# araray/sygnals

Hardware: AMD Instinct MI355X
Metric: Msamples/s STFT->MFCC (n_fft=2048, hop=512) (higher is better)
Workload: dtype f32; 1 GPU; C2: 1024 x 1 s @ 48 kHz clips per GPU, STFT n_fft=2048 hop=512 hann center -> 40-band Slaney mel -> power_to_db(ref=max, top_db=80) -> 13 MFCC (DCT-II ortho); clips_per_gpu=1024, clip_samples=48000, sr=48000, n_fft=2048, hop=512, n_mels=40, n_mfcc=13, rows_per_clip=13, parallelism=clip-sharded x1

## Files before the change

### sygnals_amd/core/features/manager.py

```python
from __future__ import annotations

import logging
from typing import Any, Dict, List, Optional

import numpy as np
import torch

from ... import _tables as T
from ... import ops
from ..._lib import SygnalsHipError

logger = logging.getLogger(__name__)

_SPECTRUM_BASED = ("spectral_centroid", "spectral_bandwidth", "spectral_flatness", "spectral_rolloff",
                   "dominant_frequency")
_SPECTROGRAM_BASED = ("spectral_contrast",)
_MELSPEC_BASED = ("mfcc",)
_FRAME_BASED = ("mean_amplitude", "std_dev_amplitude", "skewness", "kurtosis", "peak_amplitude", "crest_factor",
                "signal_entropy", "zero_crossing_rate", "rms_energy")
_REFERENCE_ONLY = ("hnr", "jitter", "shimmer")
_DEVICE_FEATURES = set(_SPECTRUM_BASED) | set(_SPECTROGRAM_BASED) | set(_MELSPEC_BASED) | set(_FRAME_BASED)
_ALL_KNOWN_FEATURES = _DEVICE_FEATURES | set(_REFERENCE_ONLY)


# ... 193 lines not shown
    if features != ["all"]:
        unknown = [f for f in features if f not in _ALL_KNOWN_FEATURES]
        if unknown:
            raise ValueError(f"Unknown feature(s) requested: {unknown}. Available: {sorted(_ALL_KNOWN_FEATURES)}")
    if y.ndim != 1:
        raise ValueError("Input audio signal 'y' must be a 1D array.")
    if output_format not in ("dataframe", "dict_of_arrays"):
        raise ValueError(f"Unsupported output format: {output_format}. Choose 'dataframe' or 'dict_of_arrays'.")
    import pandas as pd
    empty = pd.DataFrame() if output_format == "dataframe" else {"time": np.array([], dtype=np.float64)}
    if ops.num_frames(len(y), frame_length, hop_length, center) <= 0:
        logger.warning("Signal is too short for the given frame/hop length and centering setting. No frames generated.")
        return empty
    res = extract_features_batch(y[None, :].astype(np.float32), sr, features, frame_length, hop_length, center, window,
                                 feature_params)
    final = {"time": res.pop("time")}
    for k, v in res.items():
        final[k] = np.asarray(v[0], dtype=np.float64)
    if len(final) <= 1:
        logger.warning("No features were successfully extracted or passed final checks.")
        return empty if output_format == "dataframe" else {"time": final["time"]}
    if output_format == "dict_of_arrays":
        return final
    idx = pd.to_timedelta(final.pop("time"), unit="s")
    df = pd.DataFrame(final, index=idx)
    df.index.name = "time"
    return df


def features_one_launch(y, sr, hop_length, center, window, n_mels, fmin, fmax, n_mfcc, smask, roll_percent, bw_p, cplan):
    if not (1 <= n_mfcc <= n_mels <= 127 and (smask or cplan is not None)):
        return None
    launch = ops.stft2048_features_tri(y, sr, hop_length, center, window, n_mels, fmin, fmax, n_mfcc, smask, roll_percent,
                                       bw_p, cplan)
    return launch() if launch else None


TRI_FEATURES_DEFAULT = True


def feature_block(y, sr: int, hop_length: int = 512, n_mels: int = 40, n_mfcc: int = 13, roll_percent: float = 0.85,
                  n_bands: int = 6, fmin_contrast: float = 200.0, quantile: float = 0.02, out=None, one_launch=None,
                  projection: str = "auto", tri_waves: int = 16):
    ops.require_gpu()
    B, L = y.shape
    Tn = ops.num_frames(L, 2048, hop_length, True)
    freqs = np.fft.rfftfreq(2048, 1.0 / sr)
    cplan = ops._cached(("cplan", float(sr), n_bands, float(fmin_contrast), float(quantile)),
                        lambda: T.contrast_plan(freqs, sr, n_bands, fmin_contrast, quantile))
    R = int(cplan[0])
    if out is None:
        out = torch.empty((B, n_mfcc + 2 + R, Tn), dtype=torch.float32, device=y.device)
    if one_launch not in (None, True, False, "segments"):
        raise ValueError("one_launch must be None, True, False or 'segments'")
    launch = None
    if one_launch or (one_launch is None and TRI_FEATURES_DEFAULT):
        stats = torch.empty((B, 8, Tn), dtype=torch.float32, device=y.device)
        launch = ops.stft2048_features_tri(y, sr, hop_length, True, "hann", n_mels, 0.0, None, n_mfcc, 1 | 8, roll_percent, 2.0,
                                           cplan, out, stats)
        if launch is None and one_launch:
            raise SygnalsHipError("feature_block: no one-launch form for this shape (two-pass piece table + the clip's mel matrix in LDS)")
    if launch:
        _, stats, cpv = launch()
        mel = dct = None
    else:
        mel, stats, cpv = ops.stft2048_mel(y, sr, hop_length, True, "hann", 2048, n_mels, 0.0, None, 1 | 8 | 32, roll_percent,
                                           2.0, cplan, projection, tri_waves)
        dct = ops.dct_dev(n_mfcc, n_mels)
    ops._call("syg_feature_block_f32", ops._ptr(mel), B, n_mels, Tn, ops._ptr(dct), n_mfcc, 1e-10, 80.0, ops._ptr(stats),
              float(sr) / 2048.0, ops._ptr(cpv), R, 1e-10, 80.0, ops._ptr(out))
    return out


def feature_block_dominant(y, sr, hop_length, n_mels, n_mfcc):
    cplan = T.contrast_plan(np.fft.rfftfreq(2048, 1.0 / sr), sr)
    R = int(cplan[0])
    launch = None
    if TRI_FEATURES_DEFAULT:
        shape = (y.shape[0], n_mfcc + 2 + R, ops.num_frames(y.shape[1], 2048, hop_length, True))
        launch = ops.stft2048_features_tri(y, sr, hop_length, True, "hann", n_mels, 0.0, None, n_mfcc, 1 | 8, 0.85, 2.0, cplan,
                                           torch.empty(shape, dtype=torch.float32, device=y.device),
                                           torch.empty((shape[0], 8, shape[2]), dtype=torch.float32, device=y.device))
    if launch:
        return ("stft2048_kernel<16,2,7> (16 waves, staged tiles, per-wave mel projection by segment sums, clip-resident MFCC "
                "+ centroid + rolloff + contrast tail means)", launch, n_mfcc + 2 + 2 * R)
    return ("stft2048_kernel<16,2,1> (16 waves, staged tiles, mel + centroid + rolloff + contrast tail means)",
            lambda: ops.stft2048_mel(y, sr, hop_length, True, "hann", 2048, n_mels, 0.0, None, 1 | 8, 0.85, 2.0, cplan),
            n_mels + 3 + 2 * R)
```

### sygnals_amd/csrc/stft_mel.hip

```cpp
#include "stft_host.h"
#include <stdlib.h>

#define SETPRIO(n) __builtin_amdgcn_s_setprio(n)
#include "stft_dev.h"

typedef float syg_v2f __attribute__((ext_vector_type(2)));
__device__ syg_v2f syg_raw_buffer_load_v2f(__amdgpu_buffer_rsrc_t rs, int voffset, int soffset, int aux) __asm("llvm.amdgcn.raw.ptr.buffer.load.v2f32");

namespace syg {
namespace {

constexpr int NFFT = 2048;
constexpr int MC = 1024;
constexpr int NBIN = 1025;
constexpr int MAXW = 16;
constexpr int P_STRIDE = 1090;
constexpr int SC_COMPLEX = 528;
constexpr int TW2_STRIDE = 18;
constexpr int TW2_FLOATS = 4 * TW2_STRIDE * 2;
constexpr int TW1_FLOATS = 15 * 64 * 2;

struct MelPlan {
  int steps;
  int n_groups;
// ... 257 lines not shown

template <int WAVES>
__device__ __forceinline__ void stage_tile(const float* yb, int clip_bytes, float* stage, int s_begin, int span,
                                           bool wide, int w, int lane) {
  typedef __attribute__((address_space(3))) void* lds_ptr;
  const auto rs = __builtin_amdgcn_make_buffer_rsrc(const_cast<float*>(yb), 0, clip_bytes, 0x00020000);
  if (wide) {
    const int n = (span + 255) >> 8;
    for (int c = w; c < n; c += WAVES)
      __builtin_amdgcn_raw_ptr_buffer_load_lds(rs, (lds_ptr)(stage + c * 256), 16, (s_begin + c * 256 + lane * 4) * 4,
                                               0, 0, 0);
  } else {
    const int n = (span + 63) >> 6;
    for (int c = w; c < n; c += WAVES)
      __builtin_amdgcn_raw_ptr_buffer_load_lds(rs, (lds_ptr)(stage + c * 64), 4, (s_begin + c * 64 + lane) * 4, 0, 0,
                                               0);
  }
}
__device__ __forceinline__ MfccArgs uni(const MfccArgs& a) {
  MfccArgs u;
  u.dct = uni(a.dct); u.lifter = uni(a.lifter); u.out = uni(a.out); u.n_mfcc = uni(a.n_mfcc);
  u.ref_is_max = uni(a.ref_is_max); u.ref_value = uni(a.ref_value); u.amin = uni(a.amin); u.top_db = uni(a.top_db);
  u.tp = uni(a.tp); u.rows_per_clip = uni(a.rows_per_clip);
  return u;
}

typedef __attribute__((address_space(3))) float* lds_fptr;
#include "mel_segments.h"

template <int WAVES>
__device__ __noinline__ void clip_dct(int clipmel_addr, int red_addr, int dct_addr, MfccArgs mfv, int n_mels_v, int T_v, int b_v,
                                      int w_v, int lane, int stride_v = WAVES) {
  const MfccArgs mf = uni(mfv);
  const int n_mels = uni(n_mels_v), T = uni(T_v), w = uni(w_v), stride = uni(stride_v);
  const int64_t b = uni(b_v);
  lds_fptr clipmel = (lds_fptr)(uintptr_t)(uint32_t)uni(clipmel_addr);
  lds_fptr red = (lds_fptr)(uintptr_t)(uint32_t)uni(red_addr);
  lds_fptr dctl = (lds_fptr)(uintptr_t)(uint32_t)uni(dct_addr);
  lds_fptr lifl = dctl + mf.n_mfcc * n_mels;
  float m = red[lane & (WAVES - 1)];
  m = fmaxf(m, dpp_f<DPP_QP_1032>(m));
  m = fmaxf(m, dpp_f<DPP_QP_2301>(m));
  m = fmaxf(m, dpp_f<DPP_ROW_HALF_MIRROR>(m));
  m = fmaxf(m, dpp_f<DPP_ROW_MIRROR>(m));
  constexpr float DB_PER_LOG2 = 3.01029995663981195f;
  const float ref = mf.ref_is_max ? m : fabsf(mf.ref_value);
  const float reflog = __builtin_amdgcn_logf(fmaxf(mf.amin, ref));
  const float flo = (mf.top_db >= 0.f) ? DB_PER_LOG2 * (__builtin_amdgcn_logf(fmaxf(mf.amin, m)) - reflog) - mf.top_db
                                       : -3.4e38f;
  const int ktiles = (mf.n_mfcc + 15) >> 4, ttiles = mf.tp >> 4;
  const int f = lane & 15, g = lane >> 4;
  for (int ot = w; ot < ktiles * ttiles; ot += stride) {
    const int kt = ot / ttiles, tq = ot - kt * ttiles;
    const int krow = kt * 16 + f, tcol = tq * 16 + f;
    v4f acc = {0.f, 0.f, 0.f, 0.f};
    for (int m0 = 0; m0 < n_mels; m0 += 16) {
      float a[4], bv[4];
#pragma unroll
      for (int i = 0; i < 4; ++i) {
        const int mm = m0 + 4 * i + g;
        const bool ok = mm < n_mels;
        a[i] = (krow < mf.n_mfcc && ok) ? dctl[krow * n_mels + mm] : 0.f;
        bv[i] = ok ? clipmel[mm * mf.tp + tcol] : 1.f;
      }
#pragma unroll
      for (int i = 0; i < 4; ++i) {
        const float db = fmaxf(DB_PER_LOG2 * (__builtin_amdgcn_logf(fmaxf(mf.amin, bv[i])) - reflog), flo);
        acc = __builtin_amdgcn_mfma_f32_16x16x4f32(a[i], db, acc, 0, 0, 0);
      }
    }
#pragma unroll
    for (int r = 0; r < 4; ++r) {
      const int k = kt * 16 + 4 * g + r;
      if (k < mf.n_mfcc && tcol < T) {
        float val = acc[r];
        if (mf.lifter) val *= lifl[k];
        mf.out[(b * mf.rows_per_clip + k) * (int64_t)T + tcol] = val;
      }
    }
  }
}

constexpr int HANDOVER_ROUNDS = 1 << 16;
typedef __attribute__((address_space(3))) int* lds_ctr;
__device__ __forceinline__ int handover_load(lds_ctr c) {
  return __builtin_amdgcn_readfirstlane(__hip_atomic_load(c, __ATOMIC_ACQUIRE, __HIP_MEMORY_SCOPE_WORKGROUP));
}
template <int PRIO_BACK>
__device__ __forceinline__ bool handover_wait(lds_ctr c, int target) {
  if (handover_load(c) >= target) return true;
  if (PRIO_BACK >= 0) SETPRIO(0);
  bool ok = false;
#pragma unroll 1
  for (int r = 0; r < HANDOVER_ROUNDS && !ok; ++r) {
    __builtin_amdgcn_s_sleep(8);
    ok = handover_load(c) >= target;
  }
  if (PRIO_BACK >= 0) SETPRIO(PRIO_BACK);
  return ok;
}
__device__ __forceinline__ void handover_add(lds_ctr c, int lane) {
  if (lane == 0) __hip_atomic_fetch_add(c, 1, __ATOMIC_RELEASE, __HIP_MEMORY_SCOPE_WORKGROUP);
}

template <int WAVES, bool SLAB = true, int NPASS = 2>
struct Lds {
  static constexpr int TILE_T = WAVES;
  static constexpr int O_P = (NPASS == 4) ? 16 : 0;
  static constexpr int P_FLOATS = O_P + TILE_T * P_STRIDE + 16;
  static constexpr int SLAB_FLOATS = SLAB ? WAVES * 16 * TILE_T : 0;
  static constexpr int SEG_WORDS = NPASS * (SEGTAB_WORDS / 2);
  static constexpr int CPL_FLOATS = SLAB ? 3 * SYG_MAX_BANDS + MTAB_INTS : SEG_WORDS + 3 * SYG_MAX_BANDS;
  static constexpr int STAGE_FLOATS = (WAVES - 1) * 512 + NFFT;
  static constexpr int O_SLAB = P_FLOATS;
  static constexpr int O_TW2 = O_SLAB + SLAB_FLOATS;
  static constexpr int O_TW1 = O_TW2 + TW2_FLOATS;
  static constexpr int O_CPL = O_TW1 + TW1_FLOATS;
  static constexpr int O_WIN = O_CPL + CPL_FLOATS;
  static constexpr int O_STAGE = O_WIN + NFFT;
  static constexpr int TOTAL = O_STAGE + STAGE_FLOATS;
  static_assert(SC_COMPLEX * 2 <= P_STRIDE, "exchange scratch must fit inside a power row");
  static_assert(O_TW2 % 4 == 0 && O_WIN % 4 == 0 && O_STAGE % 4 == 0 && O_CPL % 4 == 0, "16-byte aligned LDS sections");
};

enum class Mode : int {
  Mel = 0, MelRows = 1, Complex = 2, ClipMatrix = 3, ClipSeg = 6, ClipSegRows = 7,
  TileSeg4 = 8, TileSeg4Rows = 9, TileSeg2 = 10, TileSeg2Rows = 11,
};
enum class Proj { None, Matrix, Segments };
constexpr bool X2_MEL = true;

struct ModeTraits {
  Proj proj;
  int npass;
  bool clip;
  bool rowfn;
  bool complex_out;
  bool power4;
  bool relc;
  bool freerun;
  constexpr bool seg() const { return proj == Proj::Segments; }
  constexpr bool seg_tile() const { return seg() && !clip; }
  constexpr bool x2() const { return X2_MEL && power4; }
  constexpr int clip_matrices() const { return seg() ? 2 : 1; }
};
constexpr ModeTraits mode_traits(Mode m) {
  switch (m) {
    case Mode::Mel:          return {Proj::Matrix,   2, false, false, false, true,  false, false};
    case Mode::MelRows:      return {Proj::Matrix,   2, false, true,  false, false, false, false};
    case Mode::Complex:      return {Proj::None,     2, false, false, true,  false, false, false};
    case Mode::ClipMatrix:   return {Proj::Matrix,   2, true,  false, false, true,  false, false};
    case Mode::ClipSeg:      return {Proj::Segments, 2, true,  false, false, true,  false,  true};
    case Mode::ClipSegRows:  return {Proj::Segments, 2, true,  true,  false, false, true, false};
    case Mode::TileSeg4:     return {Proj::Segments, 4, false, false, false, true,  false, false};
    case Mode::TileSeg4Rows: return {Proj::Segments, 4, false, true,  false, false, false, false};
    case Mode::TileSeg2:     return {Proj::Segments, 2, false, false, false, true,  false, false};
    case Mode::TileSeg2Rows: return {Proj::Segments, 2, false, true,  false, false, false, false};
  }
  return {};
}
template <int WAVES, Mode MODE>
using ModeLds = Lds<WAVES, !mode_traits(MODE).seg(), mode_traits(MODE).npass>;

template <int WAVES, int LOAD, Mode MODE>
__global__ __launch_bounds__(WAVES * 64, 4) void stft2048_kernel(
    const float* __restrict__ y, int64_t L, int64_t ldy, int hop, int pad, int64_t T, int tiles_per_clip,
    int64_t total_tiles, int tiles_per_wg, const float2* __restrict__ win2, const float2* __restrict__ twid,
    const float* __restrict__ wpacked, MelPlan plan, int n_mels, float* __restrict__ mel_out, float binhz,
    float roll_percent, float bw_p, int smask, float* __restrict__ stats_out, ContrastPlan cplan,
    float* __restrict__ contrast_out, float2* __restrict__ cout, int dma_wide, MfccArgs mf) {
  constexpr ModeTraits M = mode_traits(MODE);
  constexpr bool TRI = M.seg(), TRIMEL = M.seg_tile();
  constexpr int NPASS = M.npass;
  constexpr int TRI_ROW_BASE = (NPASS == 4) ? TRI4_ROW_BASE : 0;
  typedef ModeLds<WAVES, MODE> LM;
  constexpr int SEG_WORDS = LM::SEG_WORDS;
  constexpr int NTHREADS = WAVES * 64;
  constexpr int TILE_T = WAVES;
  constexpr bool COMPLEX_OUT = M.complex_out, ROWFN = M.rowfn, CLIPM = M.clip, X2 = M.x2();
  constexpr bool FREERUN = (LOAD >= 3), NOMEET = (LOAD == 4);
  static_assert(!FREERUN || (M.freerun && WAVES == 16 && TRI && CLIPM && !ROWFN), "LOAD 3 / 4: the free-running forms of the mode");
  constexpr int FLOAD = FREERUN ? 3 : LOAD;
#ifdef SYG_DEV_NO_RELC
  constexpr bool RELC = false;
#else
  constexpr bool RELC = M.relc;
#endif
  constexpr float MELSC = X2 ? 0.25f : 1.f;
  extern __shared__ __attribute__((aligned(16))) float lds[];
  float* Pbuf = lds + LM::O_P;
  float* slab = lds + LM::O_SLAB;
  float2* tw2l = reinterpret_cast<float2*>(lds + LM::O_TW2);
  float2* tw1l = reinterpret_cast<float2*>(lds + LM::O_TW1);
  int* cpl = reinterpret_cast<int*>(lds + LM::O_CPL);
  int* cplc = TRI ? cpl + SEG_WORDS : cpl;
  float2* winl = reinterpret_cast<float2*>(lds + LM::O_WIN);
  float* stage = lds + LM::O_STAGE;
  float* clipmel = lds + (LOAD == 2 ? LM::TOTAL : LM::O_STAGE);
  float* tri_red = clipmel + 2 * n_mels * mf.tp;
  float* tri_dct = tri_red + 2 * WAVES;

  const int tid = threadIdx.x, lane = tid & 63;
  const int w = __builtin_amdgcn_readfirstlane(tid >> 6);

  const int64_t tile_begin = (int64_t)blockIdx.x * tiles_per_wg;
  const int64_t tile_end = (tile_begin + tiles_per_wg < total_tiles) ? tile_begin + tiles_per_wg : total_tiles;
  if (tile_begin >= tile_end) return;

  auto clip_of = [&](int64_t tile) { return (uint32_t)tile / (uint32_t)tiles_per_clip; };
  auto t0_of = [&](int64_t tile, uint32_t cq) {
    return (int64_t)((uint32_t)tile - cq * (uint32_t)tiles_per_clip) * TILE_T;
  };
  const int span = (TILE_T - 1) * hop + NFFT;
  auto dma = [&](int64_t tile) {
    const uint32_t cq = clip_of(tile);
    int ld = lane;
    asm volatile("" : "+v"(ld));
    stage_tile<WAVES>(y + (int64_t)cq * ldy, (int)(L * 4), stage, (int)(t0_of(tile, cq) * hop) - pad, span,
                      dma_wide != 0, w, ld);
  };
  if (LOAD == 2) dma(tile_begin);

  LaneConst lc;
  init_lane_const(lc, lane, twid);
  float* prow = Pbuf + w * P_STRIDE;
  float2* sc = reinterpret_cast<float2*>(prow);
  if (tid < 64) tw2l[(tid >> 4) * TW2_STRIDE + (tid & 15)] = twid[32 * (tid >> 4) * (tid & 15)];
  for (int i = tid; i < 15 * 64; i += NTHREADS) tw1l[i] = twid[2 * (i & 63) * ((i >> 6) + 1)];
  for (int i = tid; i < NFFT / 2; i += NTHREADS) winl[i] = win2[i];
  if (CLIPM) {
    if (TRI)
      for (int i = tid; i < 2 * n_mels * mf.tp; i += NTHREADS) clipmel[i] = 0.f;
    float* dctl = TRI ? tri_dct : clipmel + n_mels * mf.tp + WAVES;
    for (int i = tid; i < mf.n_mfcc * n_mels; i += NTHREADS) dctl[i] = mf.dct[i];
    if (mf.lifter != nullptr && tid < mf.n_mfcc) dctl[mf.n_mfcc * n_mels + tid] = mf.lifter[tid];
  }

  int* mtab = cpl + 3 * SYG_MAX_BANDS;
  if (!COMPLEX_OUT) {
    for (int i = tid; i < LM::P_FLOATS + LM::SLAB_FLOATS; i += NTHREADS) lds[i] = 0.f;
    if (TRI && wpacked != nullptr) {
      const int band_bytes = (TRIMEL ? (int)T : mf.tp) * 4;
      for (int i = tid; i < SEG_WORDS; i += NTHREADS) {
        int v = reinterpret_cast<const int*>(wpacked)[i];
        if ((i & 3) == 1 && ((i >> 8) & 1) == 0 && v >= 0) v *= band_bytes;
        cpl[i] = v;
      }
    }
    if (!TRI || ROWFN) {
#pragma unroll
      for (int r = 0; r < SYG_MAX_BANDS; ++r)
        if (tid == r) { cplc[r] = cplan.lo[r]; cplc[SYG_MAX_BANDS + r] = cplan.hi[r]; cplc[2 * SYG_MAX_BANDS + r] = cplan.k[r]; }
    }
    if (!TRI)
      for (int i = tid; i < MTAB_INTS; i += NTHREADS) mtab[i] = reinterpret_cast<const int*>(wpacked)[plan.table_off + i];
  }
  if (NOMEET && tid < 8) cplc[tid] = 0;
  if (LOAD == 2) asm volatile("s_waitcnt vmcnt(0)" ::: "memory");
  __syncthreads();

  float cmax = 0.f;
  int64_t pend_b = -1;
  int cur = 0;
  bool tri_scan8 = false;
  if (TRI && wpacked != nullptr) {
    unsigned lk = 0;
#pragma unroll
    for (int p = 0; p < NPASS; ++p) lk |= (unsigned)(cpl[4 * (128 * p + lane) + 2] | cpl[4 * (128 * p + lane) + 3]);
    tri_scan8 = __builtin_amdgcn_ballot_w64((lk >> 24) != 0) != 0;
  }
  const int tri_ndct = ((mf.n_mfcc + 15) >> 4) * (mf.tp >> 4);
  const int tri_idle = (TRI && !TRIMEL) ? mf.tp - (int)T : 0;
  const bool tri_defer = TRI && !TRIMEL && tri_idle > 0 && (tri_ndct + tri_idle - 1) / (tri_idle > 0 ? tri_idle : 1) <= 3;
  const int tri_nepi = tri_defer ? tri_idle : (tri_ndct < WAVES ? tri_ndct : WAVES);
  float2 v[16];
  bool have = false;
  auto fetch = [&](int64_t tile) {
    const uint32_t cq = clip_of(tile);
    const int64_t t = t0_of(tile, cq) + w;
    have = t < T;
    int lf = lane;
    asm volatile("" : "+v"(lf));
    if (have) fetch_frame<FLOAD>(v, y + (int64_t)cq * ldy, L, t * (int64_t)hop - pad, stage + w * hop, lf);
  };
  if (LOAD == 2) {
    fetch(tile_begin);
    __syncthreads();
    if (tile_begin + 1 < tile_end) dma(tile_begin + 1);
  }
  if (FREERUN) fetch(tile_begin);
  lds_ctr hand = (lds_ctr)cplc;
  lds_ctr filled = hand, drained = hand + 2, bad = hand + 4;
  int kclip = 0;

#if SYG_DEV
  unsigned long long tacc[12] = {0, 0, 0, 0, 0, 0, 0, 0, 0, 0, 0, 0}, tprev, tmaxw[2] = {0, 0}, tw0;
  asm volatile("s_memtime %0\n\ts_waitcnt lgkmcnt(0)" : "=s"(tprev)::"memory");
#endif
#pragma unroll 1
  for (int64_t tile = tile_begin; tile < tile_end; ++tile) {
    const uint32_t cq = clip_of(tile);
    const int64_t b = cq;
    const int64_t t0 = t0_of(tile, cq);
    const int64_t t = t0 + w;
    if (LOAD < 2) fetch(tile);
    constexpr int PD = 1;
    SETPRIO(3 - PD);
    constexpr int NPRE = 7;
    const int ng = plan.steps >> 2;
    const float4* wp4w = reinterpret_cast<const float4*>(wpacked) + (int64_t)w * ng * 64;
    float4 apre[NPRE];
    if (have) {
      int lv = lane;
      asm volatile("" : "+v"(lv));
      if (RELC) init_lane_const<false>(lc, lv, twid);
      apply_window(v, winl, lv);
#if SYG_DEV
      tw0 = tacc[0];
      TICK(0, v[0].x);
      if (tacc[0] - tw0 > tmaxw[1]) tmaxw[1] = tacc[0] - tw0;
#endif
      float2 xs[2][4], xm[2][4], x512;
      wave_rfft2048<PD, X2>(v, lc, sc, tw1l, tw2l, lv, xs, xm, x512 TPASS);
      if (COMPLEX_OUT) {
        float2* o = cout + (b * T + t) * NBIN;
#pragma unroll
        for (int u = 0; u < 2; ++u)
#pragma unroll
          for (int d = 0; d < 4; ++d) {
            int k = lc.kb[u] + 256 * d;
            if (u == 0 && d >= 2 && lane == 0) k = (d == 2) ? 128 : 384;
            o[k] = xs[u][d];
            o[MC - k] = xm[u][d];
          }
        if (lane == 0) o[512] = x512;
      } else {
        int dA2 = lc.dA2, dA3 = lc.dA3;
        if (TRI && ROWFN) asm volatile("" : "+v"(dA2), "+v"(dA3));
#pragma unroll
        for (int u = 0; u < 2; ++u)
#pragma unroll
          for (int d = 0; d < 4; ++d) {
            const int off = (u == 0 && d == 2) ? dA2 : (u == 0 && d == 3) ? dA3 : 272 * d;
            prow[lc.pkb[u] + off] = fmaf(xs[u][d].x, xs[u][d].x, xs[u][d].y * xs[u][d].y);
            prow[lc.pmb[u] - off] = fmaf(xm[u][d].x, xm[u][d].x, xm[u][d].y * xm[u][d].y);
          }
        if (lane == 0) prow[ppos(512)] = fmaf(x512.x, x512.x, x512.y * x512.y);
      }
    } else if (!COMPLEX_OUT && !TRI) {
      for (int k = lane; k < P_STRIDE; k += 64) prow[k] = 0.f;
    }
    SETPRIO(0);
    if (COMPLEX_OUT) continue;
    if (TRI) {
      SETPRIO(3);
      const bool mine = (t < T);
      const bool clip_done = (t0 + TILE_T >= T);
      float* cmc = clipmel + cur * (n_mels * mf.tp);
      auto project = [&]() {
        int la = lane;
        asm volatile("" : "+v"(la)::"memory");
        wave_lds_sync();
        if (TRIMEL) {
          char* colg = reinterpret_cast<char*>(mel_out + (b * n_mels) * T + t);
          tri_project<NPASS>(prow - TRI_ROW_BASE, reinterpret_cast<const float4*>(cpl), la, tri_scan8,
                         [&](int boff, float v) { *reinterpret_cast<float*>(colg + boff) = MELSC * v; });
        } else {
          char* colb = reinterpret_cast<char*>(cmc + (int)t);
          tri_project<2>(prow, reinterpret_cast<const float4*>(cpl), la, tri_scan8, [&](int boff, float v) {
            *reinterpret_cast<float*>(colb + boff) = v;
            asm("v_max_f32_e32 %0, %0, %1" : "+v"(cmax) : "v"(v));
          });
        }
      };
      auto epilogue_args = [&](lds_ctr fill, int k) {
        MfccArgs a = mf;
        const bool ok = handover_wait<3>(fill, WAVES * ((k >> 1) + 1));
        if (!ok || handover_load(bad) != 0) { a.ref_is_max = 0; a.ref_value = a.amin = __builtin_nanf(""); }
        return a;
      };
      auto publish_max = [&]() {
        const float cm = wave_max(cmax);
        cmax = 0.f;
        if (lane == 0) tri_red[cur * WAVES + w] = cm;
      };
      const bool tri_proj = wpacked != nullptr;
#if SYG_DEV
      int tdep = lane;
      TICK(5, tdep);
#endif
      auto prefetch = [&]() {
        have = false;
        if (tile + 1 < tile_end) fetch(tile + 1);
      };
      const bool dct_behind = FREERUN && clip_done && !tri_defer && w < tri_ndct;
      if (FREERUN && mine && !dct_behind) prefetch();
      if (NOMEET && t0 == 0 && kclip >= 2 && !handover_wait<3>(drained + cur, tri_nepi * (kclip >> 1)) && lane == 0)
        __hip_atomic_store(bad, 1, __ATOMIC_RELAXED, __HIP_MEMORY_SCOPE_WORKGROUP);
      if (mine) {
        if (tri_proj) project();
      } else if (tri_defer && pend_b >= 0) {
        float* cmp = clipmel + (cur ^ 1) * (n_mels * mf.tp);
        const MfccArgs mfe = NOMEET ? epilogue_args(filled + (cur ^ 1), kclip - 1) : mf;
        clip_dct<WAVES>((int)(uintptr_t)(lds_fptr)cmp, (int)(uintptr_t)(lds_fptr)(tri_red + (cur ^ 1) * WAVES),
                        (int)(uintptr_t)(lds_fptr)tri_dct, mfe, n_mels, (int)T, (int)pend_b, w - (WAVES - tri_idle), lane, tri_idle);
        if (NOMEET) handover_add(drained + (cur ^ 1), lane);
      }
      if (FREERUN && !mine && !dct_behind) prefetch();
      float row_sres = 0.f;
      float2 row_pv = make_float2(0.f, 0.f);
      const bool row_early = (w >> 2) & 1;
      auto row_compute = [&]() {
        if (stats_out != nullptr && contrast_out != nullptr) {
          const float3 f = row_features<NBIN, 0>((lds_row)prow, lane, binhz, roll_percent, bw_p, smask, (lds_iptr)cplc,
                                                     cplan.n_rows, cplan.ascending);
          row_sres = f.x; row_pv = make_float2(f.y, f.z);
        } else {
          if (stats_out != nullptr) row_sres = row_stats<NBIN, 0>((lds_row)prow, lane, binhz, roll_percent, bw_p, smask);
          if (contrast_out != nullptr)
            row_pv = row_contrast_all<0>((lds_row)prow, lane, (lds_iptr)cplc, cplan.n_rows, cplan.ascending);
        }
      };
      TICK(6, tdep);
      if (ROWFN && mine && row_early) {
        row_compute();
        prow[lane] = row_sres; prow[64 + lane] = row_pv.x; prow[128 + lane] = row_pv.y;
      }
      if (CLIPM && clip_done) publish_max();
      TICK(7, tdep);
      if (NOMEET) {
        if (clip_done) handover_add(filled + cur, lane);
      } else if (FREERUN) {
        if (clip_done) __syncthreads();
      } else {
        asm volatile("s_waitcnt vmcnt(0)" ::: "memory");
        __syncthreads();
      }
#if SYG_DEV
      tw0 = tacc[8];
      TICK(8, tdep);
      if (tacc[8] - tw0 > tmaxw[0]) tmaxw[0] = tacc[8] - tw0;
#endif
      if (LOAD == 2) {
        have = false;
        if (tile + 1 < tile_end) fetch(tile + 1);
        __syncthreads();
      }
      TICK(9, tdep);
      if (CLIPM && clip_done) {
        if (tri_defer) pend_b = mf.n_mfcc > 0 ? (int64_t)b : pend_b;
        else if (w < tri_ndct) {
          const MfccArgs mfe = NOMEET ? epilogue_args(filled + cur, kclip) : mf;
          clip_dct<WAVES>((int)(uintptr_t)(lds_fptr)cmc, (int)(uintptr_t)(lds_fptr)(tri_red + cur * WAVES),
                          (int)(uintptr_t)(lds_fptr)tri_dct, mfe, n_mels, (int)T, (int)b, w, lane);
          if (NOMEET) handover_add(drained + cur, lane);
        }
        cur ^= 1;
        ++kclip;
      }
      if (dct_behind) prefetch();
      if (ROWFN && mine) {
        if (!row_early) row_compute();
        else { row_sres = prow[lane]; row_pv = make_float2(prow[64 + lane], prow[128 + lane]); }
        TICK(10, tdep);
        if (contrast_out != nullptr) {
          if (lane < cplan.n_rows) {
            contrast_out[((b * 2 + 0) * cplan.n_rows + lane) * T + t] = row_pv.x;
            contrast_out[((b * 2 + 1) * cplan.n_rows + lane) * T + t] = row_pv.y;
          }
        }
#if SYG_DEV
        if (stats_out != nullptr && row_sres == 12345.678f)
#else
        if (stats_out != nullptr && lane < SYG_NSTAT && ((stats_row_mask(smask) >> lane) & 1))
#endif
          stats_out[(b * SYG_NSTAT + lane) * T + t] = row_sres;
      }
      if (LOAD == 2 && tile + 2 < tile_end) dma(tile + 2);
      TICK(11, tdep);
      SETPRIO(0);
      continue;
    }
#if SYG_DEV
    int tdep = lane;
    TICK(5, tdep);
#endif
    int la = lane;
    asm volatile("" : "+v"(la)::"memory");
    const float4* wp4 = wp4w + la;
#pragma unroll
    for (int q = 0; q < NPRE; ++q) apre[q] = wp4[q * 64];
    const int pslot = mtab[w * 4 + (la >> 4)];
    asm volatile("s_waitcnt vmcnt(0)" ::: "memory");
    __syncthreads();
    TICK(6, tdep);
    if (!ROWFN) SETPRIO(3);
    if (CLIPM && pend_b >= 0) {
      if (w < ((mf.n_mfcc + 15) >> 4) * (mf.tp >> 4))
        clip_dct<WAVES>((int)(uintptr_t)(lds_fptr)clipmel, (int)(uintptr_t)(lds_fptr)(clipmel + n_mels * mf.tp),
                        (int)(uintptr_t)(lds_fptr)(clipmel + n_mels * mf.tp + WAVES), mf, n_mels, (int)T, (int)pend_b, w, lane);
      pend_b = -1;
      TICK(10, tdep);
    }

    {
      const int fr = (4 * ((la >> 2) & 3) + (la & 3)) & (TILE_T - 1);
      const float* pq = Pbuf + fr * P_STRIDE + pslot;
      float bq[4 * NPRE];
#pragma unroll
      for (int i = 0; i < 2 * NPRE; ++i) {
        const float2 v2 = reinterpret_cast<const float2*>(pq)[i];
        bq[2 * i] = v2.x; bq[2 * i + 1] = v2.y;
      }
      v4f acc = {0.f, 0.f, 0.f, 0.f}, acc2 = {0.f, 0.f, 0.f, 0.f};
#pragma unroll
      for (int q = 0; q < NPRE; ++q) {
        acc = __builtin_amdgcn_mfma_f32_4x4x1f32(apre[q].x, bq[4 * q + 0], acc, 0, 0, 0);
        acc2 = __builtin_amdgcn_mfma_f32_4x4x1f32(apre[q].y, bq[4 * q + 1], acc2, 0, 0, 0);
        acc = __builtin_amdgcn_mfma_f32_4x4x1f32(apre[q].z, bq[4 * q + 2], acc, 0, 0, 0);
        acc2 = __builtin_amdgcn_mfma_f32_4x4x1f32(apre[q].w, bq[4 * q + 3], acc2, 0, 0, 0);
      }
      acc += acc2;
      for (int q = NPRE; q < ng; ++q) {
        const float4 a4 = wp4[q * 64];
        const float* pb = pq + 4 * q;
        acc = __builtin_amdgcn_mfma_f32_4x4x1f32(a4.x, pb[0], acc, 0, 0, 0);
        acc = __builtin_amdgcn_mfma_f32_4x4x1f32(a4.y, pb[1], acc, 0, 0, 0);
        acc = __builtin_amdgcn_mfma_f32_4x4x1f32(a4.z, pb[2], acc, 0, 0, 0);
        acc = __builtin_amdgcn_mfma_f32_4x4x1f32(a4.w, pb[3], acc, 0, 0, 0);
      }
      if (4 * ((la >> 2) & 3) + (la & 3) < TILE_T) {
        float* sl = slab + (w * 4 + (la >> 4)) * (4 * TILE_T) + fr;
#pragma unroll
        for (int r = 0; r < 4; ++r) sl[r * TILE_T] = acc[r];
      }
      TICK(7, acc[0]);
    }
    constexpr bool FETCH_EARLY = (LOAD == 2);
    if (FETCH_EARLY) {
      have = false;
      if (tile + 1 < tile_end) fetch(tile + 1);
    }
    __syncthreads();
    TICK(8, tdep);
    const bool clip_done = CLIPM && (t0 + TILE_T >= T);
    constexpr bool TAIL = ROWFN;
    if (!TAIL && FETCH_EARLY && tile + 2 < tile_end) dma(tile + 2);

    auto combine = [&]() {
      constexpr int GL = 4 * TILE_T;
      constexpr int REDSHIFT = 6;
      for (int g = (w + WAVES - REDSHIFT) % WAVES; g < plan.n_groups; g += WAVES) {
        const int first = __builtin_amdgcn_readfirstlane(mtab[128 + g]);
        const int cnt = __builtin_amdgcn_readfirstlane(mtab[192 + g]);
        int lq = lane;
        asm volatile("" : "+v"(lq));
        if (GL == 64 || lq < GL) {
          const int m = lq / TILE_T, tt = lq & (TILE_T - 1);
          const float* sp = slab + first * GL + lq;
          float sum = 0.f;
          int q = 0;
          for (; q + 4 <= cnt; q += 4) {
// ... 35 lines not shown
        if (both) {
          const float3 f = row_features<NBIN, 0>((lds_row)prow, lane, binhz, roll_percent, bw_p, smask, (lds_iptr)cplc,
                                                     cplan.n_rows, cplan.ascending);
          sres = f.x; pk = f.y; vl = f.z;
        } else if (stats_out != nullptr) sres = row_stats<NBIN, 0>((lds_row)prow, lane, binhz, roll_percent, bw_p, smask);
        if (contrast_out != nullptr) {
          if (!both) {
            const float2 pv = row_contrast_all<0>((lds_row)prow, lane, (lds_iptr)cplc, cplan.n_rows, cplan.ascending);
            pk = pv.x; vl = pv.y;
          }
          if (lane < cplan.n_rows) {
            contrast_out[((b * 2 + 0) * cplan.n_rows + lane) * T + t] = pk;
            contrast_out[((b * 2 + 1) * cplan.n_rows + lane) * T + t] = vl;
          }
        }
#if SYG_DEV
        if (stats_out != nullptr && sres == 12345.678f)
#else
        if (stats_out != nullptr && lane < SYG_NSTAT && ((stats_row_mask(smask) >> lane) & 1))
#endif
          stats_out[(b * SYG_NSTAT + lane) * T + t] = sres;
      }
    }
    if (TAIL) {
      SETPRIO(0);
      TICK(11, tdep);
      combine();
      if (clip_done) publish();
      if (FETCH_EARLY && tile + 2 < tile_end) dma(tile + 2);
    }
  }
  if (TRIMEL) {
  } else if (TRI) {
    if (pend_b >= 0 && w < tri_ndct) {
      MfccArgs mfe = mf;
      if (NOMEET) {
        if (!handover_wait<-1>(filled + (cur ^ 1), WAVES * (((kclip - 1) >> 1) + 1)) || handover_load(bad) != 0) {
          mfe.ref_is_max = 0; mfe.ref_value = mfe.amin = __builtin_nanf("");
        }
      }
      clip_dct<WAVES>((int)(uintptr_t)(lds_fptr)(clipmel + (cur ^ 1) * (n_mels * mf.tp)),
                      (int)(uintptr_t)(lds_fptr)(tri_red + (cur ^ 1) * WAVES), (int)(uintptr_t)(lds_fptr)tri_dct, mfe, n_mels,
                      (int)T, (int)pend_b, w, lane);
    }
  } else if (CLIPM && pend_b >= 0) {
    __syncthreads();
    if (w < ((mf.n_mfcc + 15) >> 4) * (mf.tp >> 4))
      clip_dct<WAVES>((int)(uintptr_t)(lds_fptr)clipmel, (int)(uintptr_t)(lds_fptr)(clipmel + n_mels * mf.tp),
                      (int)(uintptr_t)(lds_fptr)(clipmel + n_mels * mf.tp + WAVES), mf, n_mels, (int)T, (int)pend_b, w, lane);
  }
#if SYG_DEV
  if (CLIPM && !TRI && lane < 12)
    mel_out[((int64_t)blockIdx.x * WAVES + w) * 16 + lane] = (float)tacc[lane] / (float)(tile_end - tile_begin);
  if (FREERUN && mel_out != nullptr && lane < 14)
    mel_out[((int64_t)blockIdx.x * WAVES + w) * 16 + lane] =
        lane < 12 ? (float)tacc[lane] / (float)(tile_end - tile_begin) : (float)(lane == 12 ? tmaxw[0] : tmaxw[1]);
  if (ROWFN && stats_out != nullptr && lane < 12)
    stats_out[((int64_t)blockIdx.x * WAVES + w) * 16 + lane] = (float)tacc[lane] / (float)(tile_end - tile_begin);
#endif
}

void persistent_grid(int64_t total_tiles, int waves, int& wgs, int& per) {
  const int n_cu = device_cu_count();
  int use_cu = n_cu;
  const int r = option(SYG_OPT_RESERVED_CUS);
  if (r > 0 && r < n_cu) use_cu = n_cu - r;
  const int64_t slots = (int64_t)use_cu * (waves == 8 ? 2 : 1);
  int64_t p = (total_tiles + slots - 1) / slots;
  if (p < 1) p = 1;
  per = (int)p;
  wgs = (int)((total_tiles + p - 1) / p);
}

int load_mode() {
  const int v = option(SYG_OPT_STFT_LOAD);
  return (v >= 0 && v <= 2) ? v : 2;
}

#if SYG_DEV
float* g_dev_timeline = nullptr;
#endif
constexpr bool FREERUN_DEFAULT = true;
constexpr bool NOMEET_DEFAULT = true;
bool freerun_ok(int hop, int64_t L, int64_t ldy, const float* y) {
  return hop % 2 == 0 && L % 2 == 0 && ldy % 2 == 0 && ((uintptr_t)y) % 8 == 0 && L < ((int64_t)1 << 28);
}

constexpr int64_t LDS_LIMIT = 160 * 1024;
constexpr int64_t clip_lds_bytes(int n_mat, int n_mels, int64_t tp, int n_mfcc, int waves) {
  return (n_mat * ((int64_t)n_mels * tp + waves) + (int64_t)n_mfcc * (n_mels + 1)) * (int64_t)sizeof(float);
}
template <Mode MODE>
int64_t clip_lds_bytes(int n_mels, int64_t T, int n_mfcc) {
  return clip_lds_bytes(mode_traits(MODE).clip_matrices(), n_mels, ((T + MAXW - 1) / MAXW) * MAXW, n_mfcc, MAXW);
}
template <class LM>
constexpr int clip_lds_fit(int64_t extra) {
  constexpr int64_t fixed = (int64_t)LM::TOTAL * sizeof(float), stage = (int64_t)LM::STAGE_FLOATS * sizeof(float);
  return fixed + extra <= LDS_LIMIT ? 2 : fixed - stage + extra <= LDS_LIMIT ? 1 : 0;
}

struct ClipArgs { const float* y; int64_t B, L, ldy; int hop, center; int64_t T; const float* window; const float* twiddle; };
struct MelArgs { const float* table; MelPlan plan; int n_mels; float* mel_out; };
struct StatArgs { float binhz, roll_percent, bw_p; int smask; float* stats_out; ContrastPlan cp; float* contrast_out; };
struct LaunchArgs { ClipArgs clip; MelArgs mel; StatArgs st; float* cout; MfccArgs mf; int load; hipStream_t stream; };
MfccArgs no_mfcc() { MfccArgs mf = {}; mf.amin = 1e-10f; mf.top_db = -1.f; return mf; }

template <int WAVES, Mode MODE>
int launch(const LaunchArgs& a) {
  constexpr ModeTraits M = mode_traits(MODE);
  typedef ModeLds<WAVES, MODE> LM;
  const ClipArgs& c = a.clip;
  MfccArgs mf = a.mf;
  const int n_mels = a.mel.n_mels;
  const int pad = c.center ? NFFT / 2 : 0;
  const int tiles = (int)((c.T + WAVES - 1) / WAVES);
  const int64_t total_tiles = c.B * tiles;
  int wgs = 0, per = 0;
  persistent_grid(total_tiles, WAVES, wgs, per);
  size_t lds = (size_t)LM::TOTAL * sizeof(float);
  int64_t clip_extra = 0;
  if (M.seg() || M.clip) mf.tp = tiles * WAVES;
  if (M.clip) {
    persistent_grid(c.B, WAVES, wgs, per);
    per *= tiles;
    if (M.x2()) { mf.amin *= 4.f; mf.ref_value *= 4.f; }
    clip_extra = clip_lds_bytes(M.clip_matrices(), n_mels, mf.tp, mf.n_mfcc, WAVES);
  }
  bool can_stage = !M.complex_out && c.hop <= 512 && c.L < ((int64_t)1 << 28);
  if (M.clip && clip_lds_fit<LM>(clip_extra) < 2) can_stage = false;
  int load = a.load;
  if (load == 2 && !can_stage) load = 1;
  const bool vec2 = (c.hop % 2 == 0) && (c.ldy % 2 == 0) && (((uintptr_t)c.y) % 8 == 0);
  if (load == 1 && !vec2) load = 0;
  if (M.freerun && WAVES == 16) {
    const int fr = option(SYG_OPT_STFT_FREERUN);
    const bool want = fr == 1 || (fr < 0 && FREERUN_DEFAULT && option(SYG_OPT_STFT_LOAD) < 0);
    if (want && freerun_ok(c.hop, c.L, c.ldy, c.y)) {
      const int meet = option(SYG_OPT_STFT_MEET);
      load = (meet == 0 || (meet < 0 && NOMEET_DEFAULT)) ? 4 : 3;
    }
  }
  if (M.clip) {
    lds = lds - (load != 2 ? (size_t)LM::STAGE_FLOATS * sizeof(float) : 0) + (size_t)clip_extra;
    SYG_REQUIRE(lds <= (size_t)LDS_LIMIT, "stft2048_mfcc: the clip's mel matrix (%d x %d) does not fit the LDS left over (%zu B > %zu B); "
                "use syg_stft2048_mel_f32 + syg_logmel_dct_f32", n_mels, mf.tp, lds, (size_t)LDS_LIMIT);
  }
  const int dma_wide = (c.hop % 4 == 0) && (pad % 4 == 0) && (c.ldy % 4 == 0) && (c.L % 4 == 0) && (((uintptr_t)c.y) % 16 == 0);
  auto kern = load == 2 ? stft2048_kernel<WAVES, 2, MODE>
                        : load == 1 ? stft2048_kernel<WAVES, 1, MODE> : stft2048_kernel<WAVES, 0, MODE>;
  if constexpr (M.freerun && WAVES == 16)
    if (load >= 3) kern = load == 4 ? stft2048_kernel<WAVES, 4, MODE> : stft2048_kernel<WAVES, 3, MODE>;
  float* mel_out = a.mel.mel_out;
#if SYG_DEV
  if (load >= 3) mel_out = g_dev_timeline;
#endif
  const size_t cap = M.clip ? (size_t)LDS_LIMIT : (size_t)LM::TOTAL * sizeof(float);
  if (const int rc = reserve_dynamic_lds("stft2048", (const void*)kern, cap)) return rc;
  hipLaunchKernelGGL(kern, dim3((unsigned)wgs), dim3(WAVES * 64), lds, a.stream, c.y, c.L, c.ldy, c.hop, pad, c.T,
                     tiles, total_tiles, per, (const float2*)c.window, (const float2*)c.twiddle, a.mel.table, a.mel.plan,
                     n_mels, mel_out, a.st.binhz, a.st.roll_percent, a.st.bw_p, a.st.smask, a.st.stats_out, a.st.cp,
                     a.st.contrast_out, (float2*)a.cout, dma_wide, mf);
  SYG_CHECK_LAUNCH("stft2048");
  return SYG_OK;
}
constexpr Mode tile_mode(Proj proj, int npass, bool rows) {
  return proj == Proj::Matrix ? (rows ? Mode::MelRows : Mode::Mel)
         : npass == 4 ? (rows ? Mode::TileSeg4Rows : Mode::TileSeg4) : (rows ? Mode::TileSeg2Rows : Mode::TileSeg2);
}
template <int WAVES, Proj PROJ, int NPASS>
int launch_tile(bool rows, const LaunchArgs& a) {
  return rows ? launch<WAVES, tile_mode(PROJ, NPASS, true)>(a) : launch<WAVES, tile_mode(PROJ, NPASS, false)>(a);
}

int fill_clip_args(const float* y, int64_t B, int64_t L, int64_t ldy, int hop, int center, int64_t T, const float* window,
                   const float* twiddle, int waves, void* stream, LaunchArgs& a) {
  if (const int rc = check_clips("stft2048", y, B, L, ldy, NFFT, hop, center, T, window, twiddle)) return rc;
  SYG_REQUIRE(B * ((T + waves - 1) / waves) < (int64_t)0x7fffffff, "stft2048: grid too large");
  a.clip = {y, B, L, ldy, hop, center, T, window, twiddle};
  a.load = load_mode(); a.stream = (hipStream_t)stream;
  return SYG_OK;
}

int fill_stat_args(const char* who, float sr, float roll_percent, float bw_p, int stats_mask, float* stats_out,
                   const int32_t* cplan_host, float* contrast_out, StatArgs& st) {
  int rc = parse_contrast_plan("stft2048", NBIN, contrast_out, cplan_host, st.cp);
  if (!rc && stats_out) rc = check_stats_args(who, sr, roll_percent, bw_p, stats_mask);
  st.binhz = sr / (float)NFFT; st.roll_percent = roll_percent; st.bw_p = bw_p; st.smask = stats_mask;
  st.stats_out = stats_out; st.contrast_out = contrast_out;
  return rc;
}

int parse_mel_plan(const char* who, const int32_t* plan_host, int n_mels, MelPlan& plan) {
  SYG_REQUIRE(plan_host[0] == 2, "%s: mel plan layout %d, this library needs layout 2 (sygnals_amd._tables.pack_mel_plan)",
              who, plan_host[0]);
  const int waves = plan_host[1];
  SYG_REQUIRE(waves == 8 || waves == 16, "%s: plan must be built for 8 or 16 waves (got %d)", who, waves);
  plan.steps = plan_host[2]; plan.n_groups = plan_host[3]; plan.table_off = plan_host[4];
  SYG_REQUIRE(n_mels >= 1 && plan.n_groups == (n_mels + 3) / 4 && plan.n_groups <= 64,
              "%s: plan has %d groups of four mel rows, n_mels=%d needs %d (at most 64)", who, plan.n_groups, n_mels,
              (n_mels + 3) / 4);
  SYG_REQUIRE(plan.steps >= 28 && plan.steps % 4 == 0 && plan.steps <= P_STRIDE, "%s: bad step count %d", who, plan.steps);
  SYG_REQUIRE(plan.table_off >= waves * plan.steps * 64 && plan.table_off % 4 == 0, "%s: bad table offset", who);
  static_assert(P_STRIDE % 2 == 0, "slot reads are 8-byte words");
  return SYG_OK;
}

constexpr int64_t CLIP_FRAMES_LIMIT = (int64_t)1 << 24;

}
}

using namespace syg;

extern "C" int syg_stft2048_mel_f32(const float* y, int64_t B, int64_t L, int64_t ldy, int hop, int center,
                                    int64_t T, const float* window, const float* twiddle, const float* wpacked,
                                    const int32_t* plan_host, int n_mels, float* mel_out, float sr,
                                    float roll_percent, float bw_p, int stats_mask, float* stats_out,
                                    const int32_t* cplan_host, float* contrast_out, void* stream) {
  SYG_REQUIRE(wpacked && plan_host && mel_out, "stft2048_mel: null pointer argument");
  LaunchArgs a = {};
  int rc = parse_mel_plan("stft2048_mel", plan_host, n_mels, a.mel.plan);
  if (rc) return rc;
  const int waves = plan_host[1];
  if ((rc = fill_clip_args(y, B, L, ldy, hop, center, T, window, twiddle, waves, stream, a))) return rc;
  if ((rc = fill_stat_args("stft2048_mel", sr, roll_percent, bw_p, stats_mask, stats_out, cplan_host, contrast_out, a.st))) return rc;
  if (stats_out && (rc = check_row_frames("stft2048_mel", T))) return rc;
  a.mel.table = wpacked; a.mel.n_mels = n_mels; a.mel.mel_out = mel_out;
  const bool rows = (stats_out != nullptr) || (contrast_out != nullptr);
  return waves == 8 ? launch_tile<8, Proj::Matrix, 2>(rows, a) : launch_tile<16, Proj::Matrix, 2>(rows, a);
}

extern "C" int syg_stft2048_mfcc_fits(int n_mels, int64_t T, int n_mfcc) {
  if (n_mels < 1 || n_mels > 16 * MAXW || T < 1 || n_mfcc < 1 || n_mfcc > n_mels) return 0;
  return clip_lds_fit<ModeLds<16, Mode::ClipMatrix>>(clip_lds_bytes<Mode::ClipMatrix>(n_mels, T, n_mfcc));
// ... 114 lines not shown
```

Before: 381,000 Msamples/s.

## Enable free-running no-meet waves for the clip-segment row-feature MFCC mode

Extends the free-running, never-meeting wave schedule (per-wave global prefetch, LDS handover counters) to the ClipSegRows mode, which also emits spectral row features. Each wave now computes and stores its contrast and stats rows directly instead of staging them through shared rows, then prefetches its next frame. The handover counters are placed after the DCT table in LDS, with 32 extra bytes reserved. The goal is to remove the staged-tile DMA and cross-wave meeting points, at the cost of more LDS, new per-wave global stores, and scheduling complexity.

After: 380,800 Msamples/s, median of 2. About the same (-0.1%).

```diff
diff --git a/sygnals_amd/core/features/manager.py b/sygnals_amd/core/features/manager.py
--- a/sygnals_amd/core/features/manager.py
+++ b/sygnals_amd/core/features/manager.py
@@ -299,7 +299,13 @@
                                            torch.empty(shape, dtype=torch.float32, device=y.device),
                                            torch.empty((shape[0], 8, shape[2]), dtype=torch.float32, device=y.device))
     if launch:
-        return ("stft2048_kernel<16,2,7> (16 waves, staged tiles, per-wave mel projection by segment sums, clip-resident MFCC "
+        fr, meet, load = (ops.get_option(k) for k in ("stft_freerun", "stft_meet", "stft_load"))
+        yc = y if y.stride(1) == 1 else y.contiguous()
+        free = ((fr == 1 or (fr < 0 and load < 0)) and meet <= 0 and
+                ops.lib().syg_stft2048_mfcc_tri_freerun(int(hop_length), int(yc.shape[1]), ops._ld(yc), ops._ptr(yc)) == 1)
+        form = "<16,4,7> (16 waves, free-running waves that never meet, frames prefetched from global memory" if free else \
+               "<16,2,7> (16 waves, staged tiles"
+        return (f"stft2048_kernel{form}, per-wave mel projection by segment sums, clip-resident MFCC "
                 "+ centroid + rolloff + contrast tail means)", launch, n_mfcc + 2 + 2 * R)
     return ("stft2048_kernel<16,2,1> (16 waves, staged tiles, mel + centroid + rolloff + contrast tail means)",
             lambda: ops.stft2048_mel(y, sr, hop_length, True, "hann", 2048, n_mels, 0.0, None, 1 | 8, 0.85, 2.0, cplan),
diff --git a/sygnals_amd/csrc/stft_mel.hip b/sygnals_amd/csrc/stft_mel.hip
--- a/sygnals_amd/csrc/stft_mel.hip
+++ b/sygnals_amd/csrc/stft_mel.hip
@@ -363,6 +363,7 @@
 }
 
 constexpr int HANDOVER_ROUNDS = 1 << 16;
+constexpr int HANDOVER_BYTES = 32;
 typedef __attribute__((address_space(3))) int* lds_ctr;
 __device__ __forceinline__ int handover_load(lds_ctr c) {
   return __builtin_amdgcn_readfirstlane(__hip_atomic_load(c, __ATOMIC_ACQUIRE, __HIP_MEMORY_SCOPE_WORKGROUP));
@@ -432,7 +433,7 @@
     case Mode::Complex:      return {Proj::None,     2, false, false, true,  false, false, false};
     case Mode::ClipMatrix:   return {Proj::Matrix,   2, true,  false, false, true,  false, false};
     case Mode::ClipSeg:      return {Proj::Segments, 2, true,  false, false, true,  false,  true};
-    case Mode::ClipSegRows:  return {Proj::Segments, 2, true,  true,  false, false, true, false};
+    case Mode::ClipSegRows:  return {Proj::Segments, 2, true,  true,  false, false, true,   true};
     case Mode::TileSeg4:     return {Proj::Segments, 4, false, false, false, true,  false, false};
     case Mode::TileSeg4Rows: return {Proj::Segments, 4, false, true,  false, false, false, false};
     case Mode::TileSeg2:     return {Proj::Segments, 2, false, false, false, true,  false, false};
@@ -460,7 +461,8 @@
   constexpr int TILE_T = WAVES;
   constexpr bool COMPLEX_OUT = M.complex_out, ROWFN = M.rowfn, CLIPM = M.clip, X2 = M.x2();
   constexpr bool FREERUN = (LOAD >= 3), NOMEET = (LOAD == 4);
-  static_assert(!FREERUN || (M.freerun && WAVES == 16 && TRI && CLIPM && !ROWFN), "LOAD 3 / 4: the free-running forms of the mode");
+  static_assert(!FREERUN || (M.freerun && WAVES == 16 && TRI && CLIPM && (!ROWFN || NOMEET)), "LOAD 3 / 4: the free-running forms of the mode");
+  constexpr bool ROWFREE = ROWFN && NOMEET;
   constexpr int FLOAD = FREERUN ? 3 : LOAD;
 #ifdef SYG_DEV_NO_RELC
   constexpr bool RELC = false;
@@ -536,7 +538,8 @@
     if (!TRI)
       for (int i = tid; i < MTAB_INTS; i += NTHREADS) mtab[i] = reinterpret_cast<const int*>(wpacked)[plan.table_off + i];
   }
-  if (NOMEET && tid < 8) cplc[tid] = 0;
+  int* handw = ROWFREE ? reinterpret_cast<int*>(tri_dct + mf.n_mfcc * (n_mels + 1)) : cplc;
+  if (NOMEET && tid < 8) handw[tid] = 0;
   if (LOAD == 2) asm volatile("s_waitcnt vmcnt(0)" ::: "memory");
   __syncthreads();
 
@@ -570,7 +573,7 @@
     if (tile_begin + 1 < tile_end) dma(tile_begin + 1);
   }
   if (FREERUN) fetch(tile_begin);
-  lds_ctr hand = (lds_ctr)cplc;
+  lds_ctr hand = (lds_ctr)handw;
   lds_ctr filled = hand, drained = hand + 2, bad = hand + 4;
   int kclip = 0;
 
@@ -675,7 +678,7 @@
         if (tile + 1 < tile_end) fetch(tile + 1);
       };
       const bool dct_behind = FREERUN && clip_done && !tri_defer && w < tri_ndct;
-      if (FREERUN && mine && !dct_behind) prefetch();
+      if (FREERUN && !ROWFREE && mine && !dct_behind) prefetch();
       if (NOMEET && t0 == 0 && kclip >= 2 && !handover_wait<3>(drained + cur, tri_nepi * (kclip >> 1)) && lane == 0)
         __hip_atomic_store(bad, 1, __ATOMIC_RELAXED, __HIP_MEMORY_SCOPE_WORKGROUP);
       if (mine) {
@@ -687,7 +690,7 @@
                         (int)(uintptr_t)(lds_fptr)tri_dct, mfe, n_mels, (int)T, (int)pend_b, w - (WAVES - tri_idle), lane, tri_idle);
         if (NOMEET) handover_add(drained + (cur ^ 1), lane);
       }
-      if (FREERUN && !mine && !dct_behind) prefetch();
+      if (FREERUN && !ROWFREE && !mine && !dct_behind) prefetch();
       float row_sres = 0.f;
       float2 row_pv = make_float2(0.f, 0.f);
       const bool row_early = (w >> 2) & 1;
@@ -703,7 +706,26 @@
         }
       };
       TICK(6, tdep);
-      if (ROWFN && mine && row_early) {
+      if (ROWFREE) {
+        if (mine) {
+          row_compute();
+          TICK(7, tdep);
+          if (contrast_out != nullptr) {
+            if (lane < cplan.n_rows) {
+              contrast_out[((b * 2 + 0) * cplan.n_rows + lane) * T + t] = row_pv.x;
+              contrast_out[((b * 2 + 1) * cplan.n_rows + lane) * T + t] = row_pv.y;
+            }
+          }
+#if SYG_DEV
+          if (stats_out != nullptr && row_sres == 12345.678f)
+#else
+          if (stats_out != nullptr && lane < SYG_NSTAT && ((stats_row_mask(smask) >> lane) & 1))
+#endif
+            stats_out[(b * SYG_NSTAT + lane) * T + t] = row_sres;
+        }
+        if (!dct_behind) prefetch();
+        TICK(11, tdep);
+      } else if (ROWFN && mine && row_early) {
         row_compute();
         prow[lane] = row_sres; prow[64 + lane] = row_pv.x; prow[128 + lane] = row_pv.y;
       }
@@ -740,7 +762,7 @@
         ++kclip;
       }
       if (dct_behind) prefetch();
-      if (ROWFN && mine) {
+      if (ROWFN && !ROWFREE && mine) {
         if (!row_early) row_compute();
         else { row_sres = prow[lane]; row_pv = make_float2(prow[64 + lane], prow[128 + lane]); }
         TICK(10, tdep);
@@ -758,7 +780,8 @@
           stats_out[(b * SYG_NSTAT + lane) * T + t] = row_sres;
       }
       if (LOAD == 2 && tile + 2 < tile_end) dma(tile + 2);
-      TICK(11, tdep);
+      if (ROWFREE) { TICK(10, tdep); }
+      else { TICK(11, tdep); }
       SETPRIO(0);
       continue;
     }
@@ -960,6 +983,7 @@
 #endif
 constexpr bool FREERUN_DEFAULT = true;
 constexpr bool NOMEET_DEFAULT = true;
+constexpr bool ROWFREE_DEFAULT = true;
 bool freerun_ok(int hop, int64_t L, int64_t ldy, const float* y) {
   return hop % 2 == 0 && L % 2 == 0 && ldy % 2 == 0 && ((uintptr_t)y) % 8 == 0 && L < ((int64_t)1 << 28);
 }
@@ -1013,10 +1037,16 @@
   if (load == 1 && !vec2) load = 0;
   if (M.freerun && WAVES == 16) {
     const int fr = option(SYG_OPT_STFT_FREERUN);
-    const bool want = fr == 1 || (fr < 0 && FREERUN_DEFAULT && option(SYG_OPT_STFT_LOAD) < 0);
+    const bool want = fr == 1 || (fr < 0 && (M.rowfn ? ROWFREE_DEFAULT : FREERUN_DEFAULT) && option(SYG_OPT_STFT_LOAD) < 0);
     if (want && freerun_ok(c.hop, c.L, c.ldy, c.y)) {
       const int meet = option(SYG_OPT_STFT_MEET);
-      load = (meet == 0 || (meet < 0 && NOMEET_DEFAULT)) ? 4 : 3;
+      const bool nomeet = meet == 0 || (meet < 0 && NOMEET_DEFAULT);
+      if (!M.rowfn) load = nomeet ? 4 : 3;
+      else if (nomeet && a.mel.table != nullptr &&
+               (int64_t)(LM::TOTAL - LM::STAGE_FLOATS) * (int64_t)sizeof(float) + clip_extra + HANDOVER_BYTES <= LDS_LIMIT) {
+        load = 4;
+        clip_extra += HANDOVER_BYTES;
+      }
     }
   }
   if (M.clip) {
@@ -1027,8 +1057,11 @@
   const int dma_wide = (c.hop % 4 == 0) && (pad % 4 == 0) && (c.ldy % 4 == 0) && (c.L % 4 == 0) && (((uintptr_t)c.y) % 16 == 0);
   auto kern = load == 2 ? stft2048_kernel<WAVES, 2, MODE>
                         : load == 1 ? stft2048_kernel<WAVES, 1, MODE> : stft2048_kernel<WAVES, 0, MODE>;
-  if constexpr (M.freerun && WAVES == 16)
-    if (load >= 3) kern = load == 4 ? stft2048_kernel<WAVES, 4, MODE> : stft2048_kernel<WAVES, 3, MODE>;
+  if constexpr (M.freerun && WAVES == 16) {
+    if constexpr (M.rowfn) {
+      if (load == 4) kern = stft2048_kernel<WAVES, 4, MODE>;
+    } else if (load >= 3) kern = load == 4 ? stft2048_kernel<WAVES, 4, MODE> : stft2048_kernel<WAVES, 3, MODE>;
+  }
   float* mel_out = a.mel.mel_out;
 #if SYG_DEV
   if (load >= 3) mel_out = g_dev_timeline;
```
